# Hunger-Prevails/3D-Pose-Estimation-with-Previleged-Information

Hardware: AMD Instinct MI355X
Metric: crops/sec (fwd+bwd) ResNet-50 pose head, 256x256 bs=64/GPU (higher is better)
Workload: dtype f32 (3xbf16 split, 6 products, f32 accumulate); 1 GPU; depthnet resnet50 pose head, 256x256 crops, batch 64/GPU, full step: fwd + soft-argmax + SmoothL1 + bwd + RCCL grad all-reduce + clip + Adam; global_batch=64, parallelism=dp1, dist_world_size=1, wgrad_stream_runs_beside_launch_stream=True

## Files before the change

3d-pose-estimation-with-previleged-information_amd/csrc/p3d_bn.hip:

```cpp
#include "p3d_common.h"

namespace p3d {

constexpr int BN_MAX_SPLIT = 64;

__device__ __forceinline__ void block_sum2(double& a, double& b, double* red ) {
    a = wave_sum(a);
    b = wave_sum(b);
    const int w = threadIdx.x >> 6;
    if ((threadIdx.x & 63) == 0) { red[w] = a; red[4 + w] = b; }
    __syncthreads();
    a = red[0] + red[1] + red[2] + red[3];
    b = red[4] + red[5] + red[6] + red[7];
    __syncthreads();
}

__device__ __forceinline__ float bn_shift(float beta, float mean, float sc) { return __fmaf_rn(-mean, sc, beta); }

template <bool VEC>
__global__ __launch_bounds__(256) void bn_stats_kernel(const float* __restrict__ x, double* __restrict__ partial, int N, int C, int HW) {
    const int c = blockIdx.x, s = blockIdx.y, split = gridDim.y;
    double s1 = 0.0, s2 = 0.0;
    for (int n = s; n < N; n += split) {
        const float* src = x + ((size_t)n * C + c) * HW;
// ... 274 lines not shown
                }
                if (f0 || q.x > b0 || q.x != q.x) { b0 = q.x; i0 = r * 3 + 1; f0 = false; }
                if (f0 || q.y > b0 || q.y != q.y) { b0 = q.y; i0 = r * 3 + 2; f0 = false; }
                if (f1 || q.y > b1 || q.y != q.y) { b1 = q.y; i1 = r * 3; f1 = false; }
                if (f1 || q.z > b1 || q.z != q.z) { b1 = q.z; i1 = r * 3 + 1; f1 = false; }
                if (f1 || q.w > b1 || q.w != q.w) { b1 = q.w; i1 = r * 3 + 2; f1 = false; }
            }
            const size_t o = obase + (size_t)ho * Wo + 2 * j;
            *reinterpret_cast<float2*>(y + o) = make_float2(b0, b1);
            idx[o] = (uint8_t)i0; idx[o + 1] = (uint8_t)i1;
        }
    }
}

__device__ __forceinline__ float4 stem_routed_gradient(const float* __restrict__ g, const uint8_t* __restrict__ ix, int hi, int j, int Ho, int Wo) {
    float4 acc = make_float4(0.f, 0.f, 0.f, 0.f);
    const int ho_lo = hi >> 1, ho_hi = (hi + 1) >> 1;
    for (int ho = ho_lo; ho <= ho_hi; ++ho) {
        if (ho >= Ho) continue;
        const int base = (hi - (2 * ho - 1)) * 3;
        const int row = ho * Wo + 2 * j;
        const float2 gg = *reinterpret_cast<const float2*>(g + row);
        const int k0 = ix[row], k1 = ix[row + 1];
        if (k0 == base + 1) acc.x += gg.x;
        if (k0 == base + 2) acc.y += gg.x;
        if (k1 == base) acc.y += gg.y;
        if (k1 == base + 1) acc.z += gg.y;
        if (k1 == base + 2) acc.w += gg.y;
        if (2 * j + 2 < Wo && ix[row + 2] == base) acc.w += g[row + 2];
    }
    return acc;
}

template <int PASS>
__global__ __launch_bounds__(256) void stem_bn_pool_bwd_kernel(const float* __restrict__ dyp, const uint8_t* __restrict__ idx, const float* __restrict__ x,
                                                               const float* __restrict__ gamma, const float* __restrict__ beta, const float* __restrict__ mean,
                                                               const float* __restrict__ invstd, double* __restrict__ partial, int nsplit, float* __restrict__ dx,
                                                               float* dgamma, float* dbeta, int N, int C, int H, int W, int accumulate) {
    const int c = blockIdx.x, s = blockIdx.y, split = gridDim.y;
    const int HW = H * W, Ho = H / 2, Wo = W / 2, W4 = W / 4;
    const float mu = mean[c], is = invstd[c];
    const float sc = is * gamma[c];
    const float sh = bn_shift(beta[c], mu, sc);
    double s1 = 0.0, s2 = 0.0;
    float gs = 0.f, k1 = 0.f, k2 = 0.f;
// ... 4 lines not shown
        }
        if (s == 0 && threadIdx.x == 0) {
            dbeta[c] = accumulate ? dbeta[c] + (float)s1 : (float)s1;
            dgamma[c] = accumulate ? dgamma[c] + (float)s2 : (float)s2;
        }
        gs = gamma[c] * is;
        const double cnt = (double)N * HW;
        k1 = (float)(s1 / cnt);
        k2 = (float)(s2 / cnt);
    }
    for (int n = s; n < N; n += split) {
        const size_t off = ((size_t)n * C + c) * HW;
        const float* gp = dyp + ((size_t)n * C + c) * Ho * Wo;
        const uint8_t* ix = idx + ((size_t)n * C + c) * Ho * Wo;
        const float4* xv = reinterpret_cast<const float4*>(x + off);
        for (int i = threadIdx.x; i < HW / 4; i += 256) {
            float4 g = stem_routed_gradient(gp, ix, i / W4, i % W4, Ho, Wo);
            const float4 q = xv[i];
            g.x = fmaf(q.x, sc, sh) > 0.f ? g.x : 0.f; g.y = fmaf(q.y, sc, sh) > 0.f ? g.y : 0.f;
            g.z = fmaf(q.z, sc, sh) > 0.f ? g.z : 0.f; g.w = fmaf(q.w, sc, sh) > 0.f ? g.w : 0.f;
            if constexpr (PASS == 0) {
                s1 += (double)g.x + (double)g.y + (double)g.z + (double)g.w;
                s2 += (double)(g.x * ((q.x - mu) * is)) + (double)(g.y * ((q.y - mu) * is)) + (double)(g.z * ((q.z - mu) * is)) +
                      (double)(g.w * ((q.w - mu) * is));
            } else {
                float4 d;
                d.x = gs * (g.x - k1 - (q.x - mu) * is * k2);
                d.y = gs * (g.y - k1 - (q.y - mu) * is * k2);
                d.z = gs * (g.z - k1 - (q.z - mu) * is * k2);
                d.w = gs * (g.w - k1 - (q.w - mu) * is * k2);
                reinterpret_cast<float4*>(dx + off)[i] = d;
            }
        }
    }
    if constexpr (PASS == 0) {
        __shared__ double red[8];
        block_sum2(s1, s2, red);
        if (threadIdx.x == 0) {
            partial[((size_t)c * split + s) * 2 + 0] = s1;
            partial[((size_t)c * split + s) * 2 + 1] = s2;
// ... 162 lines not shown
```

3d-pose-estimation-with-previleged-information_amd/csrc/p3d_conv.hip:

```cpp
#include "p3d_common.h"
#include "p3d_fx.h"
#include <stdlib.h>

namespace p3d {

using f32x16 = __attribute__((ext_vector_type(16))) float;

enum { MODE_FWD = 0, MODE_DGRAD = 1, MODE_WGRAD = 2 };
constexpr int OOB = (int)0x80000000;
constexpr unsigned MAX_RECORDS = 0x80000000u;
constexpr int MAX_STRIDE = 4;

struct IgemmParams {
    const float* A;
    const float* B;
    float* Cout;
    const float* bias;
    const float* ep_scale;
    const float* ep_shift;
    const float* ep_res;
    int ep_relu;
    const float* mask_in;
    const float* mult;
    int N, C, H, W, K, R, S, stride, pad, dil, Ho, Wo;
// ... 728 lines not shown
        }
        sm[(g * RS + rs) * 16 + cl] = s;
    }
    __syncthreads();
    for (int e = threadIdx.x; e < RS * 16; e += 256) {
        const int rs = e >> 4, c = e & 15;
        float s = sm[rs * 16 + c];
        for (int q = 1; q < 16; ++q) s += sm[(q * RS + rs) * 16 + c];
        tile[c * RS + rs] = s;
    }
    __syncthreads();
    float* dst = dw + (size_t)k * ldw + woff + (size_t)c0 * RS;
    for (int e = threadIdx.x; e < RS * 16; e += 256) dst[e] = accumulate ? dst[e] + tile[e] : tile[e];
}

__global__ __launch_bounds__(256) void bgrad_kernel(const float* __restrict__ dy, const float* __restrict__ mult, float* __restrict__ db, int N, int K, int HW,
                                                    int accumulate) {
    const int k = blockIdx.x;
    double s = 0.0;
    for (int n = 0; n < N; ++n) {
        const float* src = dy + ((size_t)n * K + k) * HW;
        if (mult) {
            const float* mu = mult + (size_t)n * HW;
            for (int i = threadIdx.x; i < HW; i += blockDim.x) s += mu[i] > 0.f ? src[i] : 0.f;
        } else {
            for (int i = threadIdx.x; i < HW; i += blockDim.x) s += src[i];
        }
    }
    __shared__ double red[4];
    s = wave_sum(s);
    if ((threadIdx.x & 63) == 0) red[threadIdx.x >> 6] = s;
    __syncthreads();
    if (threadIdx.x == 0) {
        const float v = (float)(red[0] + red[1] + red[2] + red[3]);
        db[k] = accumulate ? db[k] + v : v;
    }
}

__global__ __launch_bounds__(256) void mask_count_kernel(const float* __restrict__ mask, float* __restrict__ mult, float* __restrict__ mask_out,
                                                         int N, int H, int W, int R, int S, int stride, int pad, int dil, int Ho, int Wo) {
    const size_t total = (size_t)N * Ho * Wo;
    const float win = (float)(R * S);
    for (size_t i = (size_t)blockIdx.x * blockDim.x + threadIdx.x; i < total; i += (size_t)gridDim.x * blockDim.x) {
        const int n = (int)(i / (Ho * Wo));
        const int pp = (int)(i - (size_t)n * Ho * Wo);
        const int ho = pp / Wo, wo = pp - ho * Wo;
        const float* mb = mask + (size_t)n * H * W;
        float cnt = 0.f;
        for (int r = 0; r < R; ++r) {
            const int hi = ho * stride - pad + r * dil;
            if ((unsigned)hi >= (unsigned)H) continue;
// ... 524 lines not shown
    else launch_igemm<MODE_WGRAD>(pl.cfg, pl.tapm, masked, p, pl.splits, (hipStream_t)stream, wv);
    if (int32_t e = check_launch("conv2d_wgrad")) return e;
    return wgrad_finish(d, (float*)workspace, pl.splits, pl.tapm, dw, (hipStream_t)stream);
}

int32_t p3d_x3_enable(int32_t on) { return fx_set_enabled(on); }
void p3d_fx_tune(int32_t what, int32_t value) { fx_tune(what, value); }

void p3d_conv_path_stats(uint64_t* counts, double* flops, int32_t reset) {
    unsigned long long c[6];
    fx_stats(c, flops, reset);
    if (counts) for (int i = 0; i < 6; ++i) counts[i] = c[i];
}

int32_t p3d_conv2d_bgrad(const float* dy, int32_t N, int32_t K, int32_t HW, float* db, int32_t accumulate, void* stream) {
    P3D_REQUIRE(dy && db && N > 0 && K > 0 && HW > 0, "conv2d_bgrad: bad argument");
    hipLaunchKernelGGL(bgrad_kernel, dim3(K), dim3(256), 0, (hipStream_t)stream, dy, (const float*)nullptr, db, N, K, HW, accumulate);
    return check_launch("conv2d_bgrad");
}

int32_t p3d_conv2d_bgrad_masked(const float* dy, const float* mult, int32_t N, int32_t K, int32_t HW, float* db, int32_t accumulate, void* stream) {
    P3D_REQUIRE(dy && mult && db && N > 0 && K > 0 && HW > 0, "conv2d_bgrad_masked: bad argument");
    hipLaunchKernelGGL(bgrad_kernel, dim3(K), dim3(256), 0, (hipStream_t)stream, dy, mult, db, N, K, HW, accumulate);
    return check_launch("conv2d_bgrad_masked");
}

int32_t p3d_mask_count_fwd(const p3d_conv_desc* d, const float* mask, float* mult, float* mask_out, void* stream) {
    if (int32_t e = validate(d)) return e;
    P3D_REQUIRE(mask && mult && mask_out, "mask_count_fwd: null tensor");
    const int64_t total = (int64_t)d->N * d->Ho * d->Wo;
    const unsigned blocks = (unsigned)(ceil_div(total, 256) < 2048 ? ceil_div(total, 256) : 2048);
    hipLaunchKernelGGL(mask_count_kernel, dim3(blocks), dim3(256), 0, (hipStream_t)stream, mask, mult, mask_out, d->N, d->H, d->W,
                       d->R, d->S, d->stride, d->pad, d->dil, d->Ho, d->Wo);
    return check_launch("mask_count_fwd");
}

int32_t p3d_nonzero_mask(const float* x, float* mask, int64_t n, void* stream) {
    P3D_REQUIRE(x && mask && n > 0, "nonzero_mask: bad argument");
// ... 7 lines not shown
```

3d-pose-estimation-with-previleged-information_amd/csrc/p3d_fx.hip:

```cpp
#include <type_traits>
#include <mutex>
#include "p3d_common.h"
#include "p3d_fx.h"

namespace p3d {

using bf8 = __bf16 __attribute__((ext_vector_type(8)));
using f32x16 = float __attribute__((ext_vector_type(16)));
using f32x4 = float __attribute__((ext_vector_type(4)));
using f32x2 = float __attribute__((ext_vector_type(2)));
using u32x2 = unsigned __attribute__((ext_vector_type(2)));
using s4t = short __attribute__((ext_vector_type(4)));
using s8v = short __attribute__((ext_vector_type(8)));
using i32x4 = int __attribute__((ext_vector_type(4)));

constexpr int FX_BM = 128, FX_BN = 128, FX_BK = 16;
constexpr int FX_PIECE = 128 * FX_BK * 2;

using bf16x2 = __bf16 __attribute__((ext_vector_type(2)));
__device__ __forceinline__ unsigned fx_pack2(float a, float b) {
    const bf16x2 h = __builtin_convertvector(f32x2{a, b}, bf16x2);
    return __builtin_bit_cast(unsigned, h);
}
__device__ __forceinline__ void fx_split2(float x0, float x1, unsigned& hp, unsigned& mp, unsigned& lp) {
// ... 1521 lines not shown
static bool fx_masked_on() { static const bool on = [] { const char* e = getenv("P3D_FX_MASKED"); return !(e && atoi(e) == 0); }(); return on; }
bool fx_fwd_masked_applies(const p3d_conv_desc* d) { return fx_masked_on() && fx_fwd_applies(d, 64); }
bool fx_fwd_masked_any_applies(const p3d_conv_desc* d) { return fx_masked_on() && fx_fwd_any_applies(d, 64); }
bool fx_dgrad_masked_applies(const p3d_conv_desc* d) { return fx_masked_on() && fx_dgrad_applies(d, 64); }
bool fx_wgrad_masked_applies(const p3d_conv_desc* d) { return fx_masked_on() && fx_wgrad_applies(d, 96); }
size_t fx_fwd_workspace(const p3d_conv_desc* d) { return fx_plan(d, false).workspace; }
size_t fx_fwd_any_workspace(const p3d_conv_desc* d) { return fx_plan(d, false, true).workspace; }
size_t fx_dgrad_workspace(const p3d_conv_desc* d) { return fx_plan(d, true).workspace; }
int fx_partial_rows_fwd(const p3d_conv_desc* d) { return fx_plan(d, false).partial_rows; }
int fx_partial_rows_dgrad(const p3d_conv_desc* d) { return fx_plan(d, true).partial_rows; }
size_t fx_wgrad_workspace(const p3d_conv_desc* d) {
    const int a = fx_wgrad_splits(d, false), b = fx_wgrad_splits(d, true);
    return (size_t)(a > b ? a : b) * d->K * d->C * d->R * d->S * sizeof(float);
}

__device__ __forceinline__ void fx_weight_image_chunks(const float* __restrict__ w, unsigned char* __restrict__ img, int K, int C, int RS, bool bwd, size_t first, size_t step,
                                                       int ctot, int coff, const float* __restrict__ scale = nullptr) {
    const int rows = bwd ? C : K, red = bwd ? K : C;
    const int tiles = (rows + 127) / 128, ksteps = red / FX_BK;
    const size_t total = (size_t)RS * tiles * ksteps * 256;
    for (size_t i = first; i < total; i += step) {
        const int half = (int)(i & 1), row = (int)((i >> 1) & 127);
        size_t j = i >> 8;
        const int ks = (int)(j % ksteps); j /= ksteps;
        const int tm = (int)(j % tiles);
        const int tap = (int)(j / tiles);
        const int m = tm * 128 + row, k0 = ks * FX_BK + half * 8;
        unsigned hi[8], mid[8], lo[8];
#pragma unroll
        for (int e = 0; e < 8; ++e) {
            float x = 0.f;
            if (m < rows) x = bwd ? w[((size_t)(k0 + e) * ctot + coff + m) * RS + tap] : w[((size_t)m * ctot + coff + k0 + e) * RS + tap];
            if (scale && m < rows) x = x * scale[m];
            const unsigned hb = __builtin_bit_cast(unsigned, x) & 0xFFFF0000u;
            const float r1 = x - __builtin_bit_cast(float, hb);
            const unsigned mb = __builtin_bit_cast(unsigned, r1) & 0xFFFF0000u;
            const float r2 = r1 - __builtin_bit_cast(float, mb);
            hi[e] = hb; mid[e] = mb; lo[e] = __builtin_bit_cast(unsigned, r2) & 0xFFFF0000u;
        }
        unsigned char* dst = img + (((size_t)tap * tiles + tm) * ksteps + ks) * (3 * FX_PIECE) + fx_rc_off(row, half);
        *reinterpret_cast<i32x4*>(dst) = i32x4{(int)((hi[0] >> 16) | hi[1]), (int)((hi[2] >> 16) | hi[3]), (int)((hi[4] >> 16) | hi[5]), (int)((hi[6] >> 16) | hi[7])};
        *reinterpret_cast<i32x4*>(dst + FX_PIECE) = i32x4{(int)((mid[0] >> 16) | mid[1]), (int)((mid[2] >> 16) | mid[3]), (int)((mid[4] >> 16) | mid[5]), (int)((mid[6] >> 16) | mid[7])};
        *reinterpret_cast<i32x4*>(dst + 2 * FX_PIECE) = i32x4{(int)((lo[0] >> 16) | lo[1]), (int)((lo[2] >> 16) | lo[3]), (int)((lo[4] >> 16) | lo[5]), (int)((lo[6] >> 16) | lo[7])};
    }
}
__global__ __launch_bounds__(256) void fx_weight_images_kernel(const float* __restrict__ w, unsigned char* __restrict__ img_fwd, unsigned char* __restrict__ img_bwd, int K,
                                                               int C, int RS, int ctot, int coff) {
    const bool bwd = blockIdx.y == 1;
    unsigned char* img = bwd ? img_bwd : img_fwd;
    if (img) fx_weight_image_chunks(w, img, K, C, RS, bwd, (size_t)blockIdx.x * 256 + threadIdx.x, (size_t)gridDim.x * 256, ctot, coff);
}
struct FxImageJob { const float* w; unsigned char* fwd; unsigned char* bwd; int K, C, RS, pad; };
__global__ __launch_bounds__(256) void fx_weight_images_batched_kernel(const FxImageJob* __restrict__ jobs) {
    const FxImageJob j = jobs[blockIdx.y >> 1];
    const bool bwd = blockIdx.y & 1;
    unsigned char* img = bwd ? j.bwd : j.fwd;
    if (img) fx_weight_image_chunks(j.w, img, j.K, j.C, j.RS, bwd, (size_t)blockIdx.x * 256 + threadIdx.x, (size_t)gridDim.x * 256, j.C, 0);
}
int32_t fx_build_weight_images_batched(const void* jobs, int njobs, int blocks, hipStream_t st) {
    static_assert(sizeof(FxImageJob) == 40, "job table layout (ops_block.py builds it)");
    if (njobs <= 0) return P3D_OK;
    hipLaunchKernelGGL(fx_weight_images_batched_kernel, dim3((unsigned)(blocks < 1 ? 1 : blocks), (unsigned)(2 * njobs)), dim3(256), 0, st, (const FxImageJob*)jobs);
    return check_launch("fx_build_weight_images_batched");
}

constexpr int FX_FOLD_MAX_K = 2048;
__global__ __launch_bounds__(256) void fx_fold_bn_kernel(const p3d_fold_job* __restrict__ jobs) {
    const p3d_fold_job j = jobs[blockIdx.y];
    __shared__ float sc[FX_FOLD_MAX_K];
    if (j.K <= 0 || j.K > FX_FOLD_MAX_K || j.C <= 0 || j.RS <= 0 || j.c_offset < 0 || j.c_offset + j.C > j.c_total || (j.kind == 0 && j.C % FX_BK != 0) ||
        (j.kind == 2 && (j.reserved < j.C || j.reserved % 8 != 0)) || (j.kind == 3 && (j.reserved < j.C || j.reserved % 32 != 0))) return;
    const bool bn = j.gamma != nullptr;
// ... 497 lines not shown
```

3d-pose-estimation-with-previleged-information_amd/csrc/p3d_head.hip:

```cpp
#include "p3d_common.h"

namespace p3d {

__global__ __launch_bounds__(256) void maxpool_fwd_kernel(const float* __restrict__ x, float* __restrict__ y, uint8_t* __restrict__ idx,
                                                          int NC, int H, int W, int Ho, int Wo) {
    const size_t total = (size_t)NC * Ho * Wo;
    for (size_t i = (size_t)blockIdx.x * blockDim.x + threadIdx.x; i < total; i += (size_t)gridDim.x * blockDim.x) {
        const int wo = (int)(i % Wo);
        const int ho = (int)((i / Wo) % Ho);
        const size_t nc = i / ((size_t)Wo * Ho);
        const float* src = x + nc * H * W;
        float best = -INFINITY;
        int bi = 0;
        bool first = true;
#pragma unroll
        for (int r = 0; r < 3; ++r) {
            const int hi = 2 * ho - 1 + r;
            if ((unsigned)hi >= (unsigned)H) continue;
#pragma unroll
            for (int s = 0; s < 3; ++s) {
                const int wi = 2 * wo - 1 + s;
                if ((unsigned)wi >= (unsigned)W) continue;
                const float v = src[hi * W + wi];
                if (first || v > best || v != v) { best = v; bi = r * 3 + s; first = false; }
// ... 180 lines not shown
        sz += (double)(e * grid_at(d, D));
    }
    s = wave_sum(s); sx = wave_sum(sx); sy = wave_sum(sy); sz = wave_sum(sz);
    if ((t & 63) == 0) { const int w = t >> 6; red[w] = s; red[4 + w] = sx; red[8 + w] = sy; red[12 + w] = sz; }
    __syncthreads();
    HeadStats r;
    r.mx = mx;
    r.sum = red[0] + red[1] + red[2] + red[3];
    r.sx = red[4] + red[5] + red[6] + red[7];
    r.sy = red[8] + red[9] + red[10] + red[11];
    r.sz = red[12] + red[13] + red[14] + red[15];
    __syncthreads();
    return r;
}

__global__ __launch_bounds__(256) void softargmax3d_fwd_kernel(const float* __restrict__ z, float* __restrict__ coords, int D, int J, int H, int W,
                                                               float depth_range) {
    __shared__ double red[16];
    __shared__ float redf[4];
    const int b = blockIdx.x / J, j = blockIdx.x % J;
    const float* zb = z + ((size_t)b * D * J + j) * H * W;
    const HeadStats st = head_stats(zb, D, J, H, W, red, redf);
    if (threadIdx.x == 0) {
        float* o = coords + ((size_t)b * J + j) * 3;
        o[0] = (float)(st.sx / st.sum) * depth_range;
        o[1] = (float)(st.sy / st.sum) * depth_range;
        o[2] = (float)(st.sz / st.sum) * depth_range;
    }
}

__global__ __launch_bounds__(256) void softargmax3d_bwd_kernel(const float* __restrict__ dcoords, const float* __restrict__ z, float* __restrict__ dz,
                                                               int D, int J, int H, int W, float depth_range) {
    __shared__ double red[16];
    __shared__ float redf[4];
    const int b = blockIdx.x / J, j = blockIdx.x % J;
    const size_t zoff = ((size_t)b * D * J + j) * H * W;
    const float* zb = z + zoff;
    float* dzb = dz + zoff;
    const HeadStats st = head_stats(zb, D, J, H, W, red, redf);
    const float inv = (float)(1.0 / st.sum);
    const float ex = (float)(st.sx / st.sum), ey = (float)(st.sy / st.sum), ez = (float)(st.sz / st.sum);
    const float* dc = dcoords + ((size_t)b * J + j) * 3;
    const float gx = dc[0] * depth_range, gy = dc[1] * depth_range, gz = dc[2] * depth_range;
    const int HW = H * W, total = D * HW;
    for (int i = threadIdx.x; i < total; i += 256) {
        const int d = i / HW, hw = i - d * HW;
        const int h = hw / W, w = hw - h * W;
        const size_t a = (size_t)d * J * HW + hw;
        const float p = expf(zb[a] - st.mx) * inv;
        dzb[a] = p * (gx * (grid_at(w, W) - ex) + gy * (grid_at(h, H) - ey) + gz * (grid_at(d, D) - ez));
    }
}

__global__ __launch_bounds__(256) void pose_loss_kernel(const float* __restrict__ relat, const float* __restrict__ true_cam,
                                                        const uint8_t* __restrict__ true_val, float* __restrict__ loss, float* __restrict__ spec_cam,
                                                        float* __restrict__ drelat, int B, int J, int key, float loss_div, int criterion,
                                                        float loss_scale, const float* __restrict__ count_override) {
    __shared__ double red[8];
    const int t = threadIdx.x;
    const int BJ = B * J;
    double cnt = 0.0, acc = 0.0;
    for (int i = t; i < BJ; i += 256) cnt += true_val[i] ? 3.0 : 0.0;
    cnt = wave_sum(cnt);
    if ((t & 63) == 0) red[t >> 6] = cnt;
    __syncthreads();
    cnt = red[0] + red[1] + red[2] + red[3];
    __syncthreads();
    const float denom = (count_override != nullptr && count_override[0] > 0.f) ? count_override[0] : (float)(cnt > 0.0 ? cnt : 1.0);
    for (int i = t; i < BJ * 3; i += 256) {
        const int bj = i / 3, a = i - bj * 3;
        const int b = bj / J;
        const size_t ko = ((size_t)b * J + key) * 3 + a;
        const float spec = relat[i] - relat[ko] + true_cam[ko];
        spec_cam[i] = spec;
        float per = 0.f, dper = 0.f;
        if (true_val[bj]) {
            const float diff = spec / loss_div - true_cam[i] / loss_div;
            const float ad = fabsf(diff);
            if (criterion == 0) {
                if (ad < 1.f) { per = 0.5f * diff * diff; dper = diff; }
                else { per = ad - 0.5f; dper = diff > 0.f ? 1.f : -1.f; }
            } else if (criterion == 1) {
                per = ad; dper = diff > 0.f ? 1.f : (diff < 0.f ? -1.f : 0.f);
            } else {
                per = diff * diff; dper = 2.f * diff;
            }
        }
        acc += per;
        drelat[i] = dper * loss_scale / (loss_div * denom);
    }
    acc = wave_sum(acc);
    if ((t & 63) == 0) red[t >> 6] = acc;
    __syncthreads();
    if (t == 0) loss[0] = (float)((red[0] + red[1] + red[2] + red[3]) / denom);
    __syncthreads();
    for (int i = t; i < B * 3; i += 256) {
        const int b = i / 3, a = i - b * 3;
        float s = 0.f;
        for (int j = 0; j < J; ++j) s += drelat[((size_t)b * J + j) * 3 + a];
        const size_t ko = ((size_t)b * J + key) * 3 + a;
        drelat[ko] -= s;
    }
}

__global__ __launch_bounds__(256) void masked_loss_kernel(const float* __restrict__ pred, const float* __restrict__ target, const uint8_t* __restrict__ valid,
                                                          float* __restrict__ loss, float* __restrict__ dpred, int rows, int C, int criterion,
                                                          const float* __restrict__ count_override) {
    __shared__ double red[8];
    const int t = threadIdx.x;
    double cnt = 0.0, acc = 0.0;
    for (int i = t; i < rows; i += 256) cnt += valid[i] ? (double)C : 0.0;
// ... 213 lines not shown
    if (W % 4 == 0 && ((uintptr_t)dx & 15) == 0 && ((uintptr_t)dy & 7) == 0) {
        const int64_t total4 = (int64_t)NC * H * (W / 4);
        const unsigned blocks4 = (unsigned)(ceil_div(total4, 256) < 16384 ? ceil_div(total4, 256) : 16384);
        hipLaunchKernelGGL(maxpool_bwd4_kernel, dim3(blocks4), dim3(256), 0, (hipStream_t)stream, dy, idx, dx, NC, H, W, Ho, Wo);
        return check_launch("maxpool_bwd");
    }
    const int64_t total = (int64_t)NC * H * W;
    const unsigned blocks = (unsigned)(ceil_div(total, 256) < 8192 ? ceil_div(total, 256) : 8192);
    hipLaunchKernelGGL(maxpool_bwd_kernel, dim3(blocks), dim3(256), 0, (hipStream_t)stream, dy, idx, dx, NC, H, W, Ho, Wo);
    return check_launch("maxpool_bwd");
}

int32_t p3d_softargmax3d_fwd(const float* z, float* coords, int32_t B, int32_t D, int32_t J, int32_t H, int32_t W,
                             float depth_range, void* stream) {
    P3D_REQUIRE(z && coords && B > 0 && D > 0 && J > 0 && H > 0 && W > 0, "softargmax3d_fwd: bad argument");
    hipLaunchKernelGGL(softargmax3d_fwd_kernel, dim3(B * J), dim3(256), 0, (hipStream_t)stream, z, coords, D, J, H, W, depth_range);
    return check_launch("softargmax3d_fwd");
}

int32_t p3d_softargmax3d_bwd(const float* dcoords, const float* z, float* dz, int32_t B, int32_t D, int32_t J, int32_t H,
                             int32_t W, float depth_range, void* stream) {
    P3D_REQUIRE(dcoords && z && dz && B > 0 && D > 0 && J > 0 && H > 0 && W > 0, "softargmax3d_bwd: bad argument");
    hipLaunchKernelGGL(softargmax3d_bwd_kernel, dim3(B * J), dim3(256), 0, (hipStream_t)stream, dcoords, z, dz, D, J, H, W, depth_range);
    return check_launch("softargmax3d_bwd");
}

int32_t p3d_pose_loss_fwd_bwd(const float* relat, const float* true_cam, const uint8_t* true_val, float* loss, float* spec_cam,
                              float* drelat, int32_t B, int32_t J, int32_t key_index, float loss_div, int32_t criterion,
                              float loss_scale, const float* count_override, void* stream) {
    P3D_REQUIRE(relat && true_cam && true_val && loss && spec_cam && drelat, "pose_loss: null tensor");
    P3D_REQUIRE(B > 0 && J > 0 && key_index >= 0 && key_index < J, "pose_loss: bad shape B=%d J=%d key=%d", B, J, key_index);
    P3D_REQUIRE(criterion >= 0 && criterion <= 2 && loss_div != 0.f, "pose_loss: bad criterion/loss_div");
    hipLaunchKernelGGL(pose_loss_kernel, dim3(1), dim3(256), 0, (hipStream_t)stream, relat, true_cam, true_val, loss, spec_cam, drelat, B, J,
                       key_index, loss_div, criterion, loss_scale, count_override);
    return check_launch("pose_loss");
}

int32_t p3d_masked_loss_fwd_bwd(const float* pred, const float* target, const uint8_t* valid, float* loss, float* dpred, int32_t rows, int32_t C,
                                int32_t criterion, const float* count_override, void* stream) {
    P3D_REQUIRE(pred && target && valid && loss && dpred && rows > 0 && C > 0, "masked_loss: bad argument");
    P3D_REQUIRE(criterion >= 0 && criterion <= 2, "masked_loss: bad criterion %d", criterion);
    hipLaunchKernelGGL(masked_loss_kernel, dim3(1), dim3(256), 0, (hipStream_t)stream, pred, target, valid, loss, dpred, rows, C, criterion, count_override);
    return check_launch("masked_loss");
}

int32_t p3d_pose_eval_stats(const float* spec_cam, const float* true_cam, const float* rotate, const uint8_t* true_val, const int32_t* mirror,
                            int32_t B, int32_t J, float solid, float close, float rough, const float* loss, double* row, float* spec_rot_out,
                            void* stream) {
// ... 24 lines not shown
```

Before: 2302 crops/s.

## Optimize stem BN-pool bwd, bias grad, weight-image packing, softargmax and pose loss kernels

Several unrelated kernels change at once. The stem maxpool-gradient routing becomes branchless and the stats pass processes two elements per thread. Bias-grad moves to 1024-thread blocks with float4 loads over a flattened N*HW index. Weight-image packing is batched through a shared-memory transpose tile. Softargmax keeps exponentials in registers between the stats and backward passes. The pose loss uses a 1024-thread block and a wave-only valid count. The aim is to cut memory traffic and latency in small auxiliary kernels, at the cost of more code paths, higher register and shared-memory pressure, and some edge-case risk.

Result: no change. 2316 crops/s (median of 6 runs) (+0.6%).

```diff
diff --git a/3d-pose-estimation-with-previleged-information_amd/csrc/p3d_bn.hip b/3d-pose-estimation-with-previleged-information_amd/csrc/p3d_bn.hip
--- a/3d-pose-estimation-with-previleged-information_amd/csrc/p3d_bn.hip
+++ b/3d-pose-estimation-with-previleged-information_amd/csrc/p3d_bn.hip
@@ -312,21 +312,24 @@
 }
 
 __device__ __forceinline__ float4 stem_routed_gradient(const float* __restrict__ g, const uint8_t* __restrict__ ix, int hi, int j, int Ho, int Wo) {
+    const int ho0 = hi >> 1, ho1 = (hi + 1) >> 1;
+    const bool two = ho1 != ho0 && ho1 < Ho, right = 2 * j + 2 < Wo;
+    const int row0 = ho0 * Wo + 2 * j, row1 = (two ? ho1 : ho0) * Wo + 2 * j, nb = right ? 2 : 1;
+    const int a0 = ix[row0], a1 = ix[row0 + 1], an = ix[row0 + nb];
+    const int b0 = ix[row1], b1 = ix[row1 + 1], bn = ix[row1 + nb];
+    const float2 ga = *reinterpret_cast<const float2*>(g + row0), gb = *reinterpret_cast<const float2*>(g + row1);
+    const float gan = g[row0 + nb], gbn = g[row1 + nb];
     float4 acc = make_float4(0.f, 0.f, 0.f, 0.f);
-    const int ho_lo = hi >> 1, ho_hi = (hi + 1) >> 1;
-    for (int ho = ho_lo; ho <= ho_hi; ++ho) {
-        if (ho >= Ho) continue;
-        const int base = (hi - (2 * ho - 1)) * 3;
-        const int row = ho * Wo + 2 * j;
-        const float2 gg = *reinterpret_cast<const float2*>(g + row);
-        const int k0 = ix[row], k1 = ix[row + 1];
-        if (k0 == base + 1) acc.x += gg.x;
-        if (k0 == base + 2) acc.y += gg.x;
-        if (k1 == base) acc.y += gg.y;
-        if (k1 == base + 1) acc.z += gg.y;
-        if (k1 == base + 2) acc.w += gg.y;
-        if (2 * j + 2 < Wo && ix[row + 2] == base) acc.w += g[row + 2];
-    }
+    auto route = [&](bool on, int base, int k0, int k1, int kn, float2 gg, float gn) {
+        acc.x = on && k0 == base + 1 ? acc.x + gg.x : acc.x;
+        acc.y = on && k0 == base + 2 ? acc.y + gg.x : acc.y;
+        acc.y = on && k1 == base ? acc.y + gg.y : acc.y;
+        acc.z = on && k1 == base + 1 ? acc.z + gg.y : acc.z;
+        acc.w = on && k1 == base + 2 ? acc.w + gg.y : acc.w;
+        acc.w = on && right && kn == base ? acc.w + gn : acc.w;
+    };
+    route(true, (hi - (2 * ho0 - 1)) * 3, a0, a1, an, ga, gan);
+    route(two, 0, b0, b1, bn, gb, gbn);
     return acc;
 }
 
@@ -361,16 +364,31 @@
         const float* gp = dyp + ((size_t)n * C + c) * Ho * Wo;
         const uint8_t* ix = idx + ((size_t)n * C + c) * Ho * Wo;
         const float4* xv = reinterpret_cast<const float4*>(x + off);
-        for (int i = threadIdx.x; i < HW / 4; i += 256) {
-            float4 g = stem_routed_gradient(gp, ix, i / W4, i % W4, Ho, Wo);
-            const float4 q = xv[i];
+        auto masked = [&](float4 g, const float4 q) {
             g.x = fmaf(q.x, sc, sh) > 0.f ? g.x : 0.f; g.y = fmaf(q.y, sc, sh) > 0.f ? g.y : 0.f;
             g.z = fmaf(q.z, sc, sh) > 0.f ? g.z : 0.f; g.w = fmaf(q.w, sc, sh) > 0.f ? g.w : 0.f;
-            if constexpr (PASS == 0) {
-                s1 += (double)g.x + (double)g.y + (double)g.z + (double)g.w;
-                s2 += (double)(g.x * ((q.x - mu) * is)) + (double)(g.y * ((q.y - mu) * is)) + (double)(g.z * ((q.z - mu) * is)) +
-                      (double)(g.w * ((q.w - mu) * is));
-            } else {
+            return g;
+        };
+        if constexpr (PASS == 0) {
+            auto sums = [&](const float4 g, const float4 q, bool on) {
+                const double t1 = (double)g.x + (double)g.y + (double)g.z + (double)g.w;
+                const double t2 = (double)(g.x * ((q.x - mu) * is)) + (double)(g.y * ((q.y - mu) * is)) + (double)(g.z * ((q.z - mu) * is)) +
+                                  (double)(g.w * ((q.w - mu) * is));
+                s1 += on ? t1 : 0.0;
+                s2 += on ? t2 : 0.0;
+            };
+            for (int i = threadIdx.x; i < HW / 4; i += 512) {
+                const bool two = i + 256 < HW / 4;
+                const int i2 = two ? i + 256 : i;
+                const float4 q = xv[i], q2 = xv[i2];
+                const float4 g = stem_routed_gradient(gp, ix, i / W4, i % W4, Ho, Wo), g2 = stem_routed_gradient(gp, ix, i2 / W4, i2 % W4, Ho, Wo);
+                sums(masked(g, q), q, true);
+                sums(masked(g2, q2), q2, two);
+            }
+        } else {
+            for (int i = threadIdx.x; i < HW / 4; i += 256) {
+                const float4 q = xv[i];
+                const float4 g = masked(stem_routed_gradient(gp, ix, i / W4, i % W4, Ho, Wo), q);
                 float4 d;
                 d.x = gs * (g.x - k1 - (q.x - mu) * is * k2);
                 d.y = gs * (g.y - k1 - (q.y - mu) * is * k2);
diff --git a/3d-pose-estimation-with-previleged-information_amd/csrc/p3d_conv.hip b/3d-pose-estimation-with-previleged-information_amd/csrc/p3d_conv.hip
--- a/3d-pose-estimation-with-previleged-information_amd/csrc/p3d_conv.hip
+++ b/3d-pose-estimation-with-previleged-information_amd/csrc/p3d_conv.hip
@@ -766,27 +766,45 @@
     for (int e = threadIdx.x; e < RS * 16; e += 256) dst[e] = accumulate ? dst[e] + tile[e] : tile[e];
 }
 
-__global__ __launch_bounds__(256) void bgrad_kernel(const float* __restrict__ dy, const float* __restrict__ mult, float* __restrict__ db, int N, int K, int HW,
-                                                    int accumulate) {
+constexpr int BGRAD_THREADS = 1024;
+template <int V>
+__global__ __launch_bounds__(BGRAD_THREADS) void bgrad_kernel(const float* __restrict__ dy, const float* __restrict__ mult, float* __restrict__ db, int N, int K, int HW,
+                                                              int accumulate) {
     const int k = blockIdx.x;
+    const unsigned per = (unsigned)(HW / V), total = (unsigned)N * per;
     double s = 0.0;
-    for (int n = 0; n < N; ++n) {
-        const float* src = dy + ((size_t)n * K + k) * HW;
-        if (mult) {
-            const float* mu = mult + (size_t)n * HW;
-            for (int i = threadIdx.x; i < HW; i += blockDim.x) s += mu[i] > 0.f ? src[i] : 0.f;
+#pragma unroll 4
+    for (unsigned i = threadIdx.x; i < total; i += BGRAD_THREADS) {
+        const unsigned n = i / per, r = i - n * per;
+        const float* src = dy + ((size_t)n * K + k) * HW + (size_t)r * V;
+        if constexpr (V == 4) {
+            float4 q = *reinterpret_cast<const float4*>(src);
+            if (mult) {
+                const float4 mu = *reinterpret_cast<const float4*>(mult + (size_t)n * HW + (size_t)r * 4);
+                q.x = mu.x > 0.f ? q.x : 0.f; q.y = mu.y > 0.f ? q.y : 0.f; q.z = mu.z > 0.f ? q.z : 0.f; q.w = mu.w > 0.f ? q.w : 0.f;
+            }
+            s += (double)q.x + (double)q.y + (double)q.z + (double)q.w;
         } else {
-            for (int i = threadIdx.x; i < HW; i += blockDim.x) s += src[i];
-        }
-    }
-    __shared__ double red[4];
+            float q = src[0];
+            if (mult) q = mult[(size_t)n * HW + r] > 0.f ? q : 0.f;
+            s += (double)q;
+        }
+    }
+    __shared__ double red[BGRAD_THREADS / 64];
     s = wave_sum(s);
     if ((threadIdx.x & 63) == 0) red[threadIdx.x >> 6] = s;
     __syncthreads();
     if (threadIdx.x == 0) {
-        const float v = (float)(red[0] + red[1] + red[2] + red[3]);
+        double a = red[0];
+        for (int w = 1; w < BGRAD_THREADS / 64; ++w) a += red[w];
+        const float v = (float)a;
         db[k] = accumulate ? db[k] + v : v;
     }
+}
+static void launch_bgrad(const float* dy, const float* mult, float* db, int N, int K, int HW, int accumulate, hipStream_t st) {
+    const bool vec = HW % 4 == 0 && (((uintptr_t)dy | (uintptr_t)mult) & 15) == 0;
+    if (vec) hipLaunchKernelGGL(bgrad_kernel<4>, dim3(K), dim3(BGRAD_THREADS), 0, st, dy, mult, db, N, K, HW, accumulate);
+    else hipLaunchKernelGGL(bgrad_kernel<1>, dim3(K), dim3(BGRAD_THREADS), 0, st, dy, mult, db, N, K, HW, accumulate);
 }
 
 __global__ __launch_bounds__(256) void mask_count_kernel(const float* __restrict__ mask, float* __restrict__ mult, float* __restrict__ mask_out,
@@ -1341,14 +1359,14 @@
 }
 
 int32_t p3d_conv2d_bgrad(const float* dy, int32_t N, int32_t K, int32_t HW, float* db, int32_t accumulate, void* stream) {
-    P3D_REQUIRE(dy && db && N > 0 && K > 0 && HW > 0, "conv2d_bgrad: bad argument");
-    hipLaunchKernelGGL(bgrad_kernel, dim3(K), dim3(256), 0, (hipStream_t)stream, dy, (const float*)nullptr, db, N, K, HW, accumulate);
+    P3D_REQUIRE(dy && db && N > 0 && K > 0 && HW > 0 && (int64_t)N * HW <= INT32_MAX, "conv2d_bgrad: bad argument");
+    launch_bgrad(dy, nullptr, db, N, K, HW, accumulate, (hipStream_t)stream);
     return check_launch("conv2d_bgrad");
 }
 
 int32_t p3d_conv2d_bgrad_masked(const float* dy, const float* mult, int32_t N, int32_t K, int32_t HW, float* db, int32_t accumulate, void* stream) {
-    P3D_REQUIRE(dy && mult && db && N > 0 && K > 0 && HW > 0, "conv2d_bgrad_masked: bad argument");
-    hipLaunchKernelGGL(bgrad_kernel, dim3(K), dim3(256), 0, (hipStream_t)stream, dy, mult, db, N, K, HW, accumulate);
+    P3D_REQUIRE(dy && mult && db && N > 0 && K > 0 && HW > 0 && (int64_t)N * HW <= INT32_MAX, "conv2d_bgrad_masked: bad argument");
+    launch_bgrad(dy, mult, db, N, K, HW, accumulate, (hipStream_t)stream);
     return check_launch("conv2d_bgrad_masked");
 }
 
diff --git a/3d-pose-estimation-with-previleged-information_amd/csrc/p3d_fx.hip b/3d-pose-estimation-with-previleged-information_amd/csrc/p3d_fx.hip
--- a/3d-pose-estimation-with-previleged-information_amd/csrc/p3d_fx.hip
+++ b/3d-pose-estimation-with-previleged-information_amd/csrc/p3d_fx.hip
@@ -1559,6 +1559,22 @@
     return (size_t)(a > b ? a : b) * d->K * d->C * d->R * d->S * sizeof(float);
 }
 
+__device__ __forceinline__ void fx_weight_chunk_store(unsigned char* __restrict__ dst_generic, const float (&x)[8]) {
+    __attribute__((address_space(1))) unsigned char* dst = (__attribute__((address_space(1))) unsigned char*)dst_generic;
+    unsigned hi[8], mid[8], lo[8];
+#pragma unroll
+    for (int e = 0; e < 8; ++e) {
+        const unsigned hb = __builtin_bit_cast(unsigned, x[e]) & 0xFFFF0000u;
+        const float r1 = x[e] - __builtin_bit_cast(float, hb);
+        const unsigned mb = __builtin_bit_cast(unsigned, r1) & 0xFFFF0000u;
+        const float r2 = r1 - __builtin_bit_cast(float, mb);
+        hi[e] = hb; mid[e] = mb; lo[e] = __builtin_bit_cast(unsigned, r2) & 0xFFFF0000u;
+    }
+    using gi32x4 = __attribute__((address_space(1))) i32x4;
+    *(gi32x4*)(dst) = i32x4{(int)((hi[0] >> 16) | hi[1]), (int)((hi[2] >> 16) | hi[3]), (int)((hi[4] >> 16) | hi[5]), (int)((hi[6] >> 16) | hi[7])};
+    *(gi32x4*)(dst + FX_PIECE) = i32x4{(int)((mid[0] >> 16) | mid[1]), (int)((mid[2] >> 16) | mid[3]), (int)((mid[4] >> 16) | mid[5]), (int)((mid[6] >> 16) | mid[7])};
+    *(gi32x4*)(dst + 2 * FX_PIECE) = i32x4{(int)((lo[0] >> 16) | lo[1]), (int)((lo[2] >> 16) | lo[3]), (int)((lo[4] >> 16) | lo[5]), (int)((lo[6] >> 16) | lo[7])};
+}
 __device__ __forceinline__ void fx_weight_image_chunks(const float* __restrict__ w, unsigned char* __restrict__ img, int K, int C, int RS, bool bwd, size_t first, size_t step,
                                                        int ctot, int coff, const float* __restrict__ scale = nullptr) {
     const int rows = bwd ? C : K, red = bwd ? K : C;
@@ -1571,22 +1587,14 @@
         const int tm = (int)(j % tiles);
         const int tap = (int)(j / tiles);
         const int m = tm * 128 + row, k0 = ks * FX_BK + half * 8;
-        unsigned hi[8], mid[8], lo[8];
+        float x[8];
 #pragma unroll
         for (int e = 0; e < 8; ++e) {
-            float x = 0.f;
-            if (m < rows) x = bwd ? w[((size_t)(k0 + e) * ctot + coff + m) * RS + tap] : w[((size_t)m * ctot + coff + k0 + e) * RS + tap];
-            if (scale && m < rows) x = x * scale[m];
-            const unsigned hb = __builtin_bit_cast(unsigned, x) & 0xFFFF0000u;
-            const float r1 = x - __builtin_bit_cast(float, hb);
-            const unsigned mb = __builtin_bit_cast(unsigned, r1) & 0xFFFF0000u;
-            const float r2 = r1 - __builtin_bit_cast(float, mb);
-            hi[e] = hb; mid[e] = mb; lo[e] = __builtin_bit_cast(unsigned, r2) & 0xFFFF0000u;
-        }
-        unsigned char* dst = img + (((size_t)tap * tiles + tm) * ksteps + ks) * (3 * FX_PIECE) + fx_rc_off(row, half);
-        *reinterpret_cast<i32x4*>(dst) = i32x4{(int)((hi[0] >> 16) | hi[1]), (int)((hi[2] >> 16) | hi[3]), (int)((hi[4] >> 16) | hi[5]), (int)((hi[6] >> 16) | hi[7])};
-        *reinterpret_cast<i32x4*>(dst + FX_PIECE) = i32x4{(int)((mid[0] >> 16) | mid[1]), (int)((mid[2] >> 16) | mid[3]), (int)((mid[4] >> 16) | mid[5]), (int)((mid[6] >> 16) | mid[7])};
-        *reinterpret_cast<i32x4*>(dst + 2 * FX_PIECE) = i32x4{(int)((lo[0] >> 16) | lo[1]), (int)((lo[2] >> 16) | lo[3]), (int)((lo[4] >> 16) | lo[5]), (int)((lo[6] >> 16) | lo[7])};
+            x[e] = 0.f;
+            if (m < rows) x[e] = bwd ? w[((size_t)(k0 + e) * ctot + coff + m) * RS + tap] : w[((size_t)m * ctot + coff + k0 + e) * RS + tap];
+            if (scale && m < rows) x[e] = x[e] * scale[m];
+        }
+        fx_weight_chunk_store(img + (((size_t)tap * tiles + tm) * ksteps + ks) * (3 * FX_PIECE) + fx_rc_off(row, half), x);
     }
 }
 __global__ __launch_bounds__(256) void fx_weight_images_kernel(const float* __restrict__ w, unsigned char* __restrict__ img_fwd, unsigned char* __restrict__ img_bwd, int K,
@@ -1595,12 +1603,77 @@
     unsigned char* img = bwd ? img_bwd : img_fwd;
     if (img) fx_weight_image_chunks(w, img, K, C, RS, bwd, (size_t)blockIdx.x * 256 + threadIdx.x, (size_t)gridDim.x * 256, ctot, coff);
 }
+constexpr int FX_WT_K = 32, FX_WT_TAPS = 9, FX_WT_RUN = (32 * FX_WT_TAPS + 63) / 64;
+using fx_gfloat = const __attribute__((address_space(1))) float;
+template <bool CONTIG>
+__device__ __forceinline__ void fx_wt_fetch(float (&r)[FX_WT_K / 4][FX_WT_RUN], const float* __restrict__ w, size_t first, size_t row_stride, int rows, int run, int RS,
+                                            int tn, int lane) {
+    fx_gfloat* gw = (fx_gfloat*)w;
+#pragma unroll
+    for (int i = 0; i < FX_WT_K / 4; ++i)
+#pragma unroll
+        for (int q = 0; q < FX_WT_RUN; ++q) {
+            const int e = lane + 64 * q;
+            size_t off = (size_t)e;
+            if constexpr (!CONTIG) { const int c = e / tn; off = (size_t)c * RS + (e - c * tn); }
+            const bool ok = 4 * i < rows && e < run;
+            const float v = gw[ok ? first + i * row_stride + off : 0];
+            r[i][q] = ok ? v : 0.f;
+        }
+}
 struct FxImageJob { const float* w; unsigned char* fwd; unsigned char* bwd; int K, C, RS, pad; };
 __global__ __launch_bounds__(256) void fx_weight_images_batched_kernel(const FxImageJob* __restrict__ jobs) {
+    __shared__ float tile[FX_WT_K * (32 * FX_WT_TAPS + 1)];
     const FxImageJob j = jobs[blockIdx.y >> 1];
-    const bool bwd = blockIdx.y & 1;
-    unsigned char* img = bwd ? j.bwd : j.fwd;
-    if (img) fx_weight_image_chunks(j.w, img, j.K, j.C, j.RS, bwd, (size_t)blockIdx.x * 256 + threadIdx.x, (size_t)gridDim.x * 256, j.C, 0);
+    const int K = j.K, C = j.C, RS = j.RS;
+    const bool do_f = j.fwd != nullptr, do_b = j.bwd != nullptr;
+    if (!do_f && !do_b) return;
+    const int tiles_f = (K + 127) / 128, ksteps_f = C / FX_BK, tiles_b = (C + 127) / 128, ksteps_b = K / FX_BK;
+    const int kext = do_f ? tiles_f * 128 : ksteps_b * FX_BK, cext = do_b ? tiles_b * 128 : ksteps_f * FX_BK;
+    const int tc = RS < FX_WT_TAPS ? RS : FX_WT_TAPS;
+    const int cg = tc == 1 ? 8 : tc == 2 ? 4 : tc <= 4 ? 2 : 1, cw = 32 * cg;
+    const int nk = (kext + FX_WT_K - 1) / FX_WT_K, nc = (cext + cw - 1) / cw, nt = (RS + tc - 1) / tc;
+    const int lane = threadIdx.x & 63, wave = threadIdx.x >> 6;
+    const int row = lane & 31, half = lane >> 5;
+    for (int u = (blockIdx.y & 1) * gridDim.x + blockIdx.x; u < nk * nc * nt; u += 2 * gridDim.x) {
+        const int ic = u % nc, ik = (u / nc) % nk, t0 = (u / (nc * nk)) * tc;
+        const int k0 = ik * FX_WT_K, c0 = ic * cw, tn = RS - t0 < tc ? RS - t0 : tc;
+        const int sk = cw * tn + 1;
+        const int live = C - c0 < cw ? (C - c0 > 0 ? C - c0 : 0) : cw;
+        float r[FX_WT_K / 4][FX_WT_RUN];
+        const size_t first = ((size_t)(k0 + wave) * C + c0) * RS + t0;
+        if (tn == RS) fx_wt_fetch<true>(r, j.w, first, (size_t)4 * C * RS, K - k0 - wave, live * tn, RS, tn, lane);
+        else fx_wt_fetch<false>(r, j.w, first, (size_t)4 * C * RS, K - k0 - wave, live * tn, RS, tn, lane);
+#pragma unroll
+        for (int i = 0; i < FX_WT_K / 4; ++i)
+#pragma unroll
+            for (int q = 0; q < FX_WT_RUN; ++q)
+                if (lane + 64 * q < cw * tn) tile[(wave + 4 * i) * sk + lane + 64 * q] = r[i][q];
+        __syncthreads();
+        for (int wt = wave; wt < 4 * cg * tn; wt += 4) {
+            const bool bwd = wt & 1;
+            const int x = (wt >> 1) % (2 * cg), tap = (wt >> 1) / (2 * cg);
+            float v[8];
+            unsigned char* dst;
+            if (!bwd) {
+                const int ks = c0 / FX_BK + x, m = k0 + row;
+                if (!do_f || ks >= ksteps_f) continue;
+                const float* s = tile + row * sk + (x * FX_BK + half * 8) * tn + tap;
+#pragma unroll
+                for (int e = 0; e < 8; ++e) v[e] = s[e * tn];
+                dst = j.fwd + (((size_t)(t0 + tap) * tiles_f + m / 128) * ksteps_f + ks) * (3 * FX_PIECE) + fx_rc_off(m & 127, half);
+            } else {
+                const int ks = k0 / FX_BK + (x & 1), m = c0 + (x >> 1) * 32 + row;
+                if (!do_b || ks >= ksteps_b || m >= tiles_b * 128) continue;
+                const float* s = tile + ((x & 1) * FX_BK + half * 8) * sk + ((x >> 1) * 32 + row) * tn + tap;
+#pragma unroll
+                for (int e = 0; e < 8; ++e) v[e] = s[e * sk];
+                dst = j.bwd + (((size_t)(t0 + tap) * tiles_b + m / 128) * ksteps_b + ks) * (3 * FX_PIECE) + fx_rc_off(m & 127, half);
+            }
+            fx_weight_chunk_store(dst, v);
+        }
+        __syncthreads();
+    }
 }
 int32_t fx_build_weight_images_batched(const void* jobs, int njobs, int blocks, hipStream_t st) {
     static_assert(sizeof(FxImageJob) == 40, "job table layout (ops_block.py builds it)");
diff --git a/3d-pose-estimation-with-previleged-information_amd/csrc/p3d_head.hip b/3d-pose-estimation-with-previleged-information_amd/csrc/p3d_head.hip
--- a/3d-pose-estimation-with-previleged-information_amd/csrc/p3d_head.hip
+++ b/3d-pose-estimation-with-previleged-information_amd/csrc/p3d_head.hip
@@ -218,13 +218,72 @@
     return r;
 }
 
+constexpr int HEAD_REG = 4;
+inline bool head_fits_registers(const float* z, int D, int H, int W) {
+    return W % 4 == 0 && (int64_t)D * H * W <= (int64_t)HEAD_REG * 1024 && ((uintptr_t)z & 15) == 0;
+}
+
+__device__ __forceinline__ HeadStats head_stats_reg(const float* __restrict__ zb, int D, int J, int H, int W, double* red , float* redf ,
+                                                    float4 (&e)[HEAD_REG]) {
+    const int HW = H * W, total4 = D * HW / 4;
+    const int t = threadIdx.x;
+#pragma unroll
+    for (int q = 0; q < HEAD_REG; ++q) {
+        const int i = 4 * (t + q * 256);
+        const int d = i / HW, hw = i - d * HW;
+        e[q] = make_float4(-INFINITY, -INFINITY, -INFINITY, -INFINITY);
+        if (t + q * 256 < total4) e[q] = *reinterpret_cast<const float4*>(zb + (size_t)d * J * HW + hw);
+    }
+    float mx = -INFINITY;
+#pragma unroll
+    for (int q = 0; q < HEAD_REG; ++q) mx = fmaxf(mx, fmaxf(fmaxf(e[q].x, e[q].y), fmaxf(e[q].z, e[q].w)));
+    mx = wave_max(mx);
+    if ((t & 63) == 0) redf[t >> 6] = mx;
+    __syncthreads();
+    mx = fmaxf(fmaxf(redf[0], redf[1]), fmaxf(redf[2], redf[3]));
+    double s = 0, sx = 0, sy = 0, sz = 0;
+#pragma unroll
+    for (int q = 0; q < HEAD_REG; ++q) {
+        const int i = 4 * (t + q * 256);
+        const int d = i / HW, hw = i - d * HW;
+        const int h = hw / W, w = hw - h * W;
+        if (t + q * 256 < total4) {
+            e[q].x = expf(e[q].x - mx); e[q].y = expf(e[q].y - mx); e[q].z = expf(e[q].z - mx); e[q].w = expf(e[q].w - mx);
+            const float gy = grid_at(h, H), gz = grid_at(d, D);
+            s += (double)e[q].x + (double)e[q].y + (double)e[q].z + (double)e[q].w;
+            sx += (double)(e[q].x * grid_at(w, W)) + (double)(e[q].y * grid_at(w + 1, W)) + (double)(e[q].z * grid_at(w + 2, W)) + (double)(e[q].w * grid_at(w + 3, W));
+            sy += (double)(e[q].x * gy) + (double)(e[q].y * gy) + (double)(e[q].z * gy) + (double)(e[q].w * gy);
+            sz += (double)(e[q].x * gz) + (double)(e[q].y * gz) + (double)(e[q].z * gz) + (double)(e[q].w * gz);
+        } else {
+            e[q] = make_float4(0.f, 0.f, 0.f, 0.f);
+        }
+    }
+    s = wave_sum(s); sx = wave_sum(sx); sy = wave_sum(sy); sz = wave_sum(sz);
+    if ((t & 63) == 0) { const int w = t >> 6; red[w] = s; red[4 + w] = sx; red[8 + w] = sy; red[12 + w] = sz; }
+    __syncthreads();
+    HeadStats r;
+    r.mx = mx;
+    r.sum = red[0] + red[1] + red[2] + red[3];
+    r.sx = red[4] + red[5] + red[6] + red[7];
+    r.sy = red[8] + red[9] + red[10] + red[11];
+    r.sz = red[12] + red[13] + red[14] + red[15];
+    return r;
+}
+
+template <bool REG>
 __global__ __launch_bounds__(256) void softargmax3d_fwd_kernel(const float* __restrict__ z, float* __restrict__ coords, int D, int J, int H, int W,
                                                                float depth_range) {
     __shared__ double red[16];
     __shared__ float redf[4];
     const int b = blockIdx.x / J, j = blockIdx.x % J;
     const float* zb = z + ((size_t)b * D * J + j) * H * W;
-    const HeadStats st = head_stats(zb, D, J, H, W, red, redf);
+    HeadStats st;
+    if constexpr (REG) {
+        float4 e[HEAD_REG];
+        st = head_stats_reg(zb, D, J, H, W, red, redf, e);
+    } else {
+        st = head_stats(zb, D, J, H, W, red, redf);
+    }
     if (threadIdx.x == 0) {
         float* o = coords + ((size_t)b * J + j) * 3;
         o[0] = (float)(st.sx / st.sum) * depth_range;
@@ -233,6 +292,7 @@
     }
 }
 
+template <bool REG>
 __global__ __launch_bounds__(256) void softargmax3d_bwd_kernel(const float* __restrict__ dcoords, const float* __restrict__ z, float* __restrict__ dz,
                                                                int D, int J, int H, int W, float depth_range) {
     __shared__ double red[16];
@@ -241,37 +301,59 @@
     const size_t zoff = ((size_t)b * D * J + j) * H * W;
     const float* zb = z + zoff;
     float* dzb = dz + zoff;
-    const HeadStats st = head_stats(zb, D, J, H, W, red, redf);
+    float4 e[HEAD_REG];
+    HeadStats st;
+    if constexpr (REG) st = head_stats_reg(zb, D, J, H, W, red, redf, e);
+    else st = head_stats(zb, D, J, H, W, red, redf);
     const float inv = (float)(1.0 / st.sum);
     const float ex = (float)(st.sx / st.sum), ey = (float)(st.sy / st.sum), ez = (float)(st.sz / st.sum);
     const float* dc = dcoords + ((size_t)b * J + j) * 3;
     const float gx = dc[0] * depth_range, gy = dc[1] * depth_range, gz = dc[2] * depth_range;
     const int HW = H * W, total = D * HW;
-    for (int i = threadIdx.x; i < total; i += 256) {
-        const int d = i / HW, hw = i - d * HW;
-        const int h = hw / W, w = hw - h * W;
-        const size_t a = (size_t)d * J * HW + hw;
-        const float p = expf(zb[a] - st.mx) * inv;
-        dzb[a] = p * (gx * (grid_at(w, W) - ex) + gy * (grid_at(h, H) - ey) + gz * (grid_at(d, D) - ez));
-    }
-}
-
-__global__ __launch_bounds__(256) void pose_loss_kernel(const float* __restrict__ relat, const float* __restrict__ true_cam,
-                                                        const uint8_t* __restrict__ true_val, float* __restrict__ loss, float* __restrict__ spec_cam,
-                                                        float* __restrict__ drelat, int B, int J, int key, float loss_div, int criterion,
-                                                        float loss_scale, const float* __restrict__ count_override) {
-    __shared__ double red[8];
+    if constexpr (REG) {
+#pragma unroll
+        for (int q = 0; q < HEAD_REG; ++q) {
+            const int i = 4 * (threadIdx.x + q * 256);
+            if (i >= total) continue;
+            const int d = i / HW, hw = i - d * HW;
+            const int h = hw / W, w = hw - h * W;
+            const float yz = gy * (grid_at(h, H) - ey), zz = gz * (grid_at(d, D) - ez);
+            float4 o;
+            o.x = (e[q].x * inv) * (gx * (grid_at(w, W) - ex) + yz + zz);
+            o.y = (e[q].y * inv) * (gx * (grid_at(w + 1, W) - ex) + yz + zz);
+            o.z = (e[q].z * inv) * (gx * (grid_at(w + 2, W) - ex) + yz + zz);
+            o.w = (e[q].w * inv) * (gx * (grid_at(w + 3, W) - ex) + yz + zz);
+            *reinterpret_cast<float4*>(dzb + (size_t)d * J * HW + hw) = o;
+        }
+    } else {
+        for (int i = threadIdx.x; i < total; i += 256) {
+            const int d = i / HW, hw = i - d * HW;
+            const int h = hw / W, w = hw - h * W;
+            const size_t a = (size_t)d * J * HW + hw;
+            const float p = expf(zb[a] - st.mx) * inv;
+            dzb[a] = p * (gx * (grid_at(w, W) - ex) + gy * (grid_at(h, H) - ey) + gz * (grid_at(d, D) - ez));
+        }
+    }
+}
+
+constexpr int POSE_LOSS_THREADS = 1024;
+__global__ __launch_bounds__(POSE_LOSS_THREADS) void pose_loss_kernel(const float* __restrict__ relat, const float* __restrict__ true_cam,
+                                                                      const uint8_t* __restrict__ true_val, float* __restrict__ loss, float* __restrict__ spec_cam,
+                                                                      float* __restrict__ drelat, int B, int J, int key, float loss_div, int criterion,
+                                                                      float loss_scale, const float* __restrict__ count_override) {
+    constexpr int T = POSE_LOSS_THREADS;
+    __shared__ double red[T / 64];
     const int t = threadIdx.x;
     const int BJ = B * J;
-    double cnt = 0.0, acc = 0.0;
-    for (int i = t; i < BJ; i += 256) cnt += true_val[i] ? 3.0 : 0.0;
-    cnt = wave_sum(cnt);
-    if ((t & 63) == 0) red[t >> 6] = cnt;
-    __syncthreads();
-    cnt = red[0] + red[1] + red[2] + red[3];
-    __syncthreads();
+    double valid = 0.0;
+#pragma unroll 4
+    for (int i = t & 63; i < BJ; i += 64) valid += true_val[i] ? 1.0 : 0.0;
+    valid = wave_sum(valid);
+    const double cnt = 3.0 * valid;
+    double acc = 0.0;
     const float denom = (count_override != nullptr && count_override[0] > 0.f) ? count_override[0] : (float)(cnt > 0.0 ? cnt : 1.0);
-    for (int i = t; i < BJ * 3; i += 256) {
+#pragma unroll 4
+    for (int i = t; i < BJ * 3; i += T) {
         const int bj = i / 3, a = i - bj * 3;
         const int b = bj / J;
         const size_t ko = ((size_t)b * J + key) * 3 + a;
@@ -296,9 +378,12 @@
     acc = wave_sum(acc);
     if ((t & 63) == 0) red[t >> 6] = acc;
     __syncthreads();
-    if (t == 0) loss[0] = (float)((red[0] + red[1] + red[2] + red[3]) / denom);
-    __syncthreads();
-    for (int i = t; i < B * 3; i += 256) {
+    if (t == 0) {
+        double sum = red[0];
+        for (int w = 1; w < T / 64; ++w) sum += red[w];
+        loss[0] = (float)(sum / denom);
+    }
+    for (int i = t; i < B * 3; i += T) {
         const int b = i / 3, a = i - b * 3;
         float s = 0.f;
         for (int j = 0; j < J; ++j) s += drelat[((size_t)b * J + j) * 3 + a];
@@ -542,14 +627,18 @@
 int32_t p3d_softargmax3d_fwd(const float* z, float* coords, int32_t B, int32_t D, int32_t J, int32_t H, int32_t W,
                              float depth_range, void* stream) {
     P3D_REQUIRE(z && coords && B > 0 && D > 0 && J > 0 && H > 0 && W > 0, "softargmax3d_fwd: bad argument");
-    hipLaunchKernelGGL(softargmax3d_fwd_kernel, dim3(B * J), dim3(256), 0, (hipStream_t)stream, z, coords, D, J, H, W, depth_range);
+    if (head_fits_registers(z, D, H, W)) hipLaunchKernelGGL(softargmax3d_fwd_kernel<true>, dim3(B * J), dim3(256), 0, (hipStream_t)stream, z, coords, D, J, H, W, depth_range);
+    else hipLaunchKernelGGL(softargmax3d_fwd_kernel<false>, dim3(B * J), dim3(256), 0, (hipStream_t)stream, z, coords, D, J, H, W, depth_range);
     return check_launch("softargmax3d_fwd");
 }
 
 int32_t p3d_softargmax3d_bwd(const float* dcoords, const float* z, float* dz, int32_t B, int32_t D, int32_t J, int32_t H,
                              int32_t W, float depth_range, void* stream) {
     P3D_REQUIRE(dcoords && z && dz && B > 0 && D > 0 && J > 0 && H > 0 && W > 0, "softargmax3d_bwd: bad argument");
-    hipLaunchKernelGGL(softargmax3d_bwd_kernel, dim3(B * J), dim3(256), 0, (hipStream_t)stream, dcoords, z, dz, D, J, H, W, depth_range);
+    if (head_fits_registers(z, D, H, W) && ((uintptr_t)dz & 15) == 0)
+        hipLaunchKernelGGL(softargmax3d_bwd_kernel<true>, dim3(B * J), dim3(256), 0, (hipStream_t)stream, dcoords, z, dz, D, J, H, W, depth_range);
+    else
+        hipLaunchKernelGGL(softargmax3d_bwd_kernel<false>, dim3(B * J), dim3(256), 0, (hipStream_t)stream, dcoords, z, dz, D, J, H, W, depth_range);
     return check_launch("softargmax3d_bwd");
 }
 
@@ -559,7 +648,7 @@
     P3D_REQUIRE(relat && true_cam && true_val && loss && spec_cam && drelat, "pose_loss: null tensor");
     P3D_REQUIRE(B > 0 && J > 0 && key_index >= 0 && key_index < J, "pose_loss: bad shape B=%d J=%d key=%d", B, J, key_index);
     P3D_REQUIRE(criterion >= 0 && criterion <= 2 && loss_div != 0.f, "pose_loss: bad criterion/loss_div");
-    hipLaunchKernelGGL(pose_loss_kernel, dim3(1), dim3(256), 0, (hipStream_t)stream, relat, true_cam, true_val, loss, spec_cam, drelat, B, J,
+    hipLaunchKernelGGL(pose_loss_kernel, dim3(1), dim3(POSE_LOSS_THREADS), 0, (hipStream_t)stream, relat, true_cam, true_val, loss, spec_cam, drelat, B, J,
                        key_index, loss_div, criterion, loss_scale, count_override);
     return check_launch("pose_loss");
 }
```
